# hsp-iit/roft

Measured on AMD Instinct MI355X. Metric: tracker frames/sec per object (640x480) + ADD-S vs CPU ref, higher is better.
Workload: dtype f64; 1 GPU; BASELINE config #4: 640x480, CV_32FC2 flow grid 1, 64 objects in total, 64 per GPU (sharded by object, no data-path collective; result rows all-gathered over RCCL at N > 1), masks+poses at 5 fps with 6-frame delay, flow-aided masks, re-sync and outlier rejection on, frames submitted in batches of at most 8; objects_per_gpu=64, objects_total=64, width=640, height=480, batch_frames=8, ranks=1, backend=nccl

## Files before the change

### include/roft_engine.h

```cpp
#ifndef ROFT_ENGINE_H
#define ROFT_ENGINE_H

#include <stddef.h>
#include <stdint.h>

#ifdef __cplusplus
extern "C" {
#endif

#define ROFT_ABI_VERSION 2

#define ROFT_OK 0
#define ROFT_ERR_INVALID (-1)
#define ROFT_ERR_DEVICE (-2)
#define ROFT_ERR_CAPACITY (-3)
#define ROFT_ERR_STATE (-4)

#define ROFT_FLOW_S16C2 11
#define ROFT_FLOW_F32C2 13

#define ROFT_MEAS_NONE 0
#define ROFT_MEAS_VELOCITY 1
#define ROFT_MEAS_POSE 2
#define ROFT_MEAS_POSE_VELOCITY 3
// ... 360 lines not shown

#define ROFT_SCENE_MAX_INSTANCES 256

typedef struct {
    int n_frames;
    int n_instances;
    const int* mesh_index;
    const double* poses;
    const uint8_t* valid;
    const uint8_t* background;
    int background_frames;
    int gray_background;
    const roft_scene_style* styles;
    int window_pixels;
} roft_scene_desc;

typedef struct roft_scene_renderer roft_scene_renderer;
int roft_scene_renderer_create(const roft_camera* cam, const roft_mesh* meshes, int n_meshes, int max_frames_per_call, int device,
                               roft_scene_renderer** out);
int roft_scene_renderer_destroy(roft_scene_renderer* r);
int roft_scene_render(roft_scene_renderer* r, const roft_scene_desc* desc, uint8_t* rgb_out, float* depth_out, int32_t* instance_out,
                      int32_t* triangle_out);
int roft_render_scene(const roft_camera* cam, const roft_mesh* meshes, int n_meshes, const roft_scene_desc* desc, uint8_t* rgb_out,
                      float* depth_out, int32_t* instance_out, int32_t* triangle_out);

int roft_debug_plan(const roft_config* cfg, const int* pose_valid, int n_frames, int* n_steps, int* n_corrections,
                    int* outlier, int* slots);
int roft_debug_restart_check(const roft_config* cfg, int n_objects, const int* has_mesh, const int* enrolled, int enrol_all,
                             const int* obj_ids, const roft_object_desc* descs, int n, int flags);
int roft_debug_probe_streams(roft_engine* e, double out[25]);
int roft_debug_sector_rate(int device, double* sectors_per_second);
int roft_debug_get_residency(roft_engine* e, unsigned long long out[32]);
int roft_debug_outlier_split(int mode);
int roft_debug_pose_errors_kernel_ms(double* ms_out);
int roft_debug_scene_kernel_ms(roft_scene_renderer* r, double ms_out[2]);
int roft_debug_depth_kernel_ms(roft_engine* e, double* ms_out);
int roft_debug_quality_kernel_ms(roft_engine* e, double* ms_out);
int roft_debug_pose_mask_kernel_ms(roft_engine* e, double* ms_out);
int roft_debug_get_dbg(roft_engine* e, int obj_id, long long out[32]);

#ifdef __cplusplus
}
#endif
#endif
```

### roft_amd/_lib.py

```python
import collections
import ctypes as C
import os
import subprocess

_HERE = os.path.dirname(os.path.abspath(__file__))
CSRC = os.path.join(_HERE, "csrc")
SO = os.environ.get("ROFT_LIB_SO") or os.path.join(CSRC, "libroft_hip.so")

OK = 0
ERR_INVALID, ERR_DEVICE, ERR_CAPACITY, ERR_STATE = -1, -2, -3, -4
FLOW_S16C2 = 11
FLOW_F32C2 = 13
MEAS_NONE, MEAS_VELOCITY, MEAS_POSE, MEAS_POSE_VELOCITY = 0, 1, 2, 3
MEM_HOST, MEM_DEVICE = 0, 1
RETAIN_FRAMES = 16
MAX_BATCH_FRAMES = 8
MAX_FLOW_CHASE = 30
RENDER_CONTRACT, RENDER_GL = 0, 1
ABI_VERSION = 2
POSE_ERROR_ADD, POSE_ERROR_ADDS = 0, 1
RESTART_KEEP_MESH = 1
LABEL_U8, LABEL_U16 = 1, 2
IMAGE_GRAY8, IMAGE_BGR8, IMAGE_RGB8 = 1, 2, 3
DEPTH_Z16 = 1
# ... 229 lines not shown
    Fn("roft_default_of_consistency", _int, [_P(OFConsistency)], _OPTIONAL),
    Fn("roft_optical_flow_checked", _int, [_vp, _vp, _int, _int, _P(OFParams), _P(OFConsistency), _vp], _OPTIONAL),
    Fn("roft_flow_producer_set_consistency", _int, [_vp, _P(OFConsistency)], _OPTIONAL),
    Fn("roft_engine_enable_flow_consistency", _int, [_vp, _P(OFConsistency)], _OPTIONAL),
    Fn("roft_engine_enable_raw_depth", _int, [_vp, _P(DepthSource)], _OPTIONAL),
    Fn("roft_engine_get_depth", _int, [_vp, _int, _vp], _OPTIONAL),
    Fn("roft_engine_get_depth_stats", _int, [_vp, _P(EngineDepthStats)], _OPTIONAL),
    Fn("roft_depth_convert", _int, [_vp, _int, _int, C.c_float, _vp], _OPTIONAL),
    Fn("roft_depth_align", _int, [_vp, _P(DepthSource), _P(Camera), _vp], _OPTIONAL),
    Fn("roft_default_quality_params", _int, [_P(QualityParams)], _OPTIONAL),
    Fn("roft_engine_enable_quality", _int, [_vp, _P(QualityParams)], _OPTIONAL),
    Fn("roft_engine_get_quality", _int, [_vp, _int, _int, _vp], _OPTIONAL),
    Fn("roft_track_quality", _int, [_P(Camera), _int, _vp, _vp, _P(Mesh), _vp, _vp, C.c_float, C.c_double, _int, _P(QualityRecord)], _OPTIONAL),
    Fn("roft_engine_enable_pose_masks", _int, [_vp, _ip, _int], _OPTIONAL),
    Fn("roft_engine_get_pose_mask_stats", _int, [_vp, _P(EnginePoseMaskStats)], _OPTIONAL),
    Fn("roft_pose_silhouette", _int, [_P(Camera), _P(Mesh), _vp, _vp, _int, _int, _vp, _ip], _OPTIONAL),
    Fn("roft_engine_enable_pose_mask_occlusion", _int, [_vp, _ip, _ip, _int], _OPTIONAL),
    Fn("roft_engine_get_pose_mask_occlusion_stats", _int, [_vp, _P(EnginePoseMaskOcclusionStats)], _OPTIONAL),
    Fn("roft_pose_silhouettes_occluded", _int, [_P(Camera), _P(Mesh), _int, _vp, _vp, _int, _int, _vp, _ip], _OPTIONAL),
    Fn("roft_default_pose_mask_gate", _int, [_P(PoseMaskGate)], _OPTIONAL),
    Fn("roft_engine_enable_pose_mask_depth_gate", _int, [_vp, _P(PoseMaskGate)], _OPTIONAL),
    Fn("roft_engine_get_pose_mask_gate_stats", _int, [_vp, _P(EnginePoseMaskGateStats)], _OPTIONAL),
    Fn("roft_pose_silhouettes_gated", _int, [_P(Camera), _P(Mesh), _int, _vp, _vp, _vp, _P(PoseMaskGate), _int, _int, _vp, _ip, _ip], _OPTIONAL),
    Fn("roft_scene_renderer_create", _int, [_P(Camera), _P(Mesh), _int, _int, _int, _P(_vp)], _OPTIONAL),
    Fn("roft_scene_renderer_destroy", _int, [_vp], _OPTIONAL),
    Fn("roft_scene_render", _int, [_vp, _P(SceneDesc), _vp, _vp, _vp, _vp], _OPTIONAL),
    Fn("roft_render_scene", _int, [_P(Camera), _P(Mesh), _int, _P(SceneDesc), _vp, _vp, _vp, _vp], _OPTIONAL),
    Fn("roft_debug_plan", _int, [_P(Config), _vp, _int, _vp, _vp, _vp, _vp], _OPTIONAL),
    Fn("roft_debug_restart_check", _int, [_P(Config), _int, _ip, _ip, _int, _ip, _P(ObjectDesc), _int, _int], _OPTIONAL),
    Fn("roft_debug_probe_streams", _int, [_vp, _dp], _OPTIONAL),
    Fn("roft_debug_sector_rate", _int, [_int, _dp], _OPTIONAL),
    Fn("roft_debug_get_residency", _int, [_vp, _P(C.c_ulonglong)], _OPTIONAL),
    Fn("roft_debug_outlier_split", _int, [_int], _OPTIONAL),
    Fn("roft_debug_pose_errors_kernel_ms", _int, [_dp], _OPTIONAL),
    Fn("roft_debug_scene_kernel_ms", _int, [_vp, _dp], _OPTIONAL),
    Fn("roft_debug_depth_kernel_ms", _int, [_vp, _dp], _OPTIONAL),
    Fn("roft_debug_quality_kernel_ms", _int, [_vp, _dp], _OPTIONAL),
    Fn("roft_debug_pose_mask_kernel_ms", _int, [_vp, _dp], _OPTIONAL),
    Fn("roft_debug_get_dbg", _int, [_vp, _int, _P(C.c_longlong)], _OPTIONAL),
)
ABI_SYMBOLS = [f.name for f in ABI]
NEWER_SYMBOLS = tuple(f.name for f in ABI if f.optional and not f.name.startswith("roft_debug_"))


def build(force=False):
    srcs = [os.path.join(CSRC, f) for f in os.listdir(CSRC) if f.endswith((".hip", ".h"))]
    srcs.append(os.path.join(_HERE, "..", "include", "roft_engine.h"))
    stale = (not os.path.exists(SO)) or any(os.path.getmtime(s) > os.path.getmtime(SO) for s in srcs)
    if force or stale:
        jobs = str(min(8, os.cpu_count() or 1))
        r = subprocess.run(["make", "-C", CSRC, "-j", jobs, "libroft_hip.so"], capture_output=True, text=True)
        if r.returncode != 0:
            raise RoftError("building libroft_hip.so failed:\n" + r.stdout[-4000:] + r.stderr[-4000:])
    return SO


_lib = None


def lib():
    global _lib
    if _lib is not None:
        return _lib
    if not os.path.exists(SO):
        build()
    L = C.CDLL(SO)
# ... 21 lines not shown
```

### roft_amd/csrc/engine_ops.hip

```cpp
#include "engine_internal.h"

namespace {

struct OpCtx {
    std::mutex mu;
    hipStream_t stream = nullptr;
    Arrays arr;
    int W = 0, H = 0, ftype = 0, fgrid = 0, radius = 0;
    DevBuf<unsigned char> b0, b1, b2, b3, b4, b5;
    DeviceMesh mesh;
    bool ready = false;

    int prepare(const roft_camera& cam, int ftype_, int fgrid_, float fscale, int radius_)
    {
        if (roft_device_count() <= 0) return fail(ROFT_ERR_DEVICE, "no HIP device (libroft_hip has no CPU path)");
        if (int rc = check_geometry(cam.width, cam.height)) return rc;
        HIP_TRY(hipSetDevice(0));
        (void)hipGetLastError();
        if (!stream) HIP_TRY(hipStreamCreateWithFlags(&stream, hipStreamNonBlocking));
        DevFlowFmt ff;
        ff.type = ftype_;
        ff.grid = std::max(fgrid_, 1);
        ff.cols = cam.width / ff.grid;
        ff.rows = cam.height / ff.grid;
// ... 544 lines not shown
    if (err != hipSuccess) { delete st; HIP_TRY(err); }
    c.arr.a.n_obj = 1;
    if (int rc = upload_ctrl(c, fc)) { delete st; return rc; }
    launch_ukf_chain(c.arr.a, *ut, true, 0, c.stream);
    err = hipMemcpyAsync(st, c.arr.state.p, sizeof(ObjState), hipMemcpyDeviceToHost, c.stream);
    if (err == hipSuccess) err = hipStreamSynchronize(c.stream);
    if (err == hipSuccess) err = hipGetLastError();
    if (err == hipSuccess) {
        std::memcpy(mean_out, st->belief[B_SPARE].mean, sizeof(double) * 13);
        std::memcpy(P_out, st->belief[B_SPARE].cov, sizeof(double) * 144);
        if (status) *status = st->lane[0].ukf_status & 0xF;
    }
    delete st;
    HIP_TRY(err);
    return ROFT_OK;
}

int roft_ukf_predict(const double mean[13], const double P[144], const double Q[81], double T, const roft_ut_params* ut,
                     double mean_out[13], double P_out[144])
{
    if (!mean || !P || !Q || !ut || !mean_out || !P_out) return fail(ROFT_ERR_INVALID, "null argument");
    return op_ukf(mean, P, Q, T, 0, nullptr, nullptr, ut, mean_out, P_out, nullptr);
}

int roft_ukf_correct(const double mean[13], const double P[144], int type, const double* meas, const double* Rdiag,
                     const roft_ut_params* ut, double mean_out[13], double P_out[144], int* status_out)
{
    if (!mean || !P || !ut || !mean_out || !P_out) return fail(ROFT_ERR_INVALID, "null argument");
    if (type != ROFT_MEAS_NONE && (!meas || !Rdiag)) return fail(ROFT_ERR_INVALID, "null measurement");
    if (type < ROFT_MEAS_NONE || type > ROFT_MEAS_POSE_VELOCITY) return fail(ROFT_ERR_INVALID, "bad measurement type");
    return op_ukf(mean, P, nullptr, 0.0, type, meas, Rdiag, ut, mean_out, P_out, status_out);
}

static int op_outlier(const roft_camera* cam, int divider, const float* depth, const uint8_t* mask, const roft_mesh* mesh,
                      const double* x2 , const double* q2 , const OutlierLaunchOpts& o_in, double L_out[2],
                      long samples_out[2], int* selected_out, float* tiles_out)
{
    TRY(check_mesh(*mesh, "mesh", false));
    OpCtx& c = op();
    std::lock_guard<std::mutex> lk(c.mu);
    if (int rc = c.prepare(*cam, ROFT_FLOW_F32C2, 1, 1.0f, 35)) return rc;
    EngineArrays& a = c.arr.a;
    a.cam.divider = divider;
    a.tile_w = cam->width / divider;
    a.tile_h = cam->height / divider;
    const size_t npix = (size_t)cam->width * cam->height, tpix = (size_t)a.tile_w * a.tile_h;
    if (int rc = c.arr.ensure_zmerge(1, tpix)) return rc;
    auto restore = [&]() {
        a.cam = make_cam(*cam);
        a.tile_w = cam->width / a.cam.divider;
        a.tile_h = cam->height / a.cam.divider;
        a.max_verts = a.max_tris = 0;
        a.meshes_without_clusters = 0;
    };
    TRY(c.mesh.upload(*mesh, o_in.render_mode == ROFT_RENDER_CONTRACT ? MeshLayout::kWalkClusters : MeshLayout::kAsItIs, c.stream));
    ObjParams prm;
    std::memset(&prm, 0, sizeof(prm));
    c.mesh.describe(prm);
    a.max_verts = mesh->n_verts;
    a.max_tris = mesh->n_tris;
    a.meshes_without_clusters = (prm.n_tris > 0 && prm.n_clusters <= 0) ? 1 : 0;
    FrameCtrl fc;
    clear_ctrl(fc);
    fc.n_steps = 1;
    fc.outlier_step = 0;
    fc.cur_slot = B_LIN0;
// ... 18 lines not shown
        PoseBelief& b = st->belief[b_alt(0, k)];
        for (int i = 0; i < 3; ++i) b.mean[6 + i] = x2[3 * k + i];
        for (int i = 0; i < 4; ++i) b.mean[9 + i] = q2[4 * k + i];
    }
    hipError_t err = hipMemcpyAsync(c.arr.state.p, st, sizeof(ObjState), hipMemcpyHostToDevice, c.stream);
    if (err == hipSuccess) err = hipMemcpyAsync(c.arr.params.p, &prm, sizeof(prm), hipMemcpyHostToDevice, c.stream);
    if (err == hipSuccess) err = hipStreamSynchronize(c.stream);
    if (err != hipSuccess) { delete st; restore(); HIP_TRY(err); }
    if (int rc = upload_ctrl(c, fc)) { delete st; restore(); return rc; }
    OutlierLaunchOpts o = o_in;
    if (tiles_out) {
        err = c.b4.ensure(sizeof(float) * 2 * tpix);
        if (err == hipSuccess) err = hipMemsetAsync(c.b4.p, 0, sizeof(float) * 2 * tpix, c.stream);
        if (err != hipSuccess) { delete st; restore(); HIP_TRY(err); }
        o.tile_dump = reinterpret_cast<float*>(c.b4.p);
    }
    if (depth && mask) {
        launch_mask_ingest(a, 0, c.stream);
        launch_features(a, c.stream);
    }
    TRY(launch_outlier(a, 0, c.stream, nullptr, &o));
    roft_ut_params ut{1.0, 2.0, 0.0};
    launch_ukf_chain(a, ut, false, 0, c.stream);
    err = hipMemcpyAsync(st, c.arr.state.p, sizeof(ObjState), hipMemcpyDeviceToHost, c.stream);
    if (err == hipSuccess && tiles_out) err = hipMemcpyAsync(tiles_out, c.b4.p, sizeof(float) * 2 * tpix, hipMemcpyDeviceToHost, c.stream);
    if (err == hipSuccess) err = hipStreamSynchronize(c.stream);
    if (err == hipSuccess) err = hipGetLastError();
    if (err == hipSuccess) {
        for (int k = 0; k < 2; ++k) {
            if (L_out) L_out[k] = st->lane[0].outlier_L[k];
            if (samples_out) samples_out[k] = (long)st->lane[0].outlier_cnt[k];
        }
        if (selected_out) *selected_out = st->lane[0].outlier_selected;
    }
    delete st;
    restore();
    HIP_TRY(err);
    return ROFT_OK;
}

int roft_mesh_classify(const roft_mesh* mesh, uint8_t* flip_out, int* closed_out)
{
    if (!mesh || !mesh->verts || !mesh->tris || !has_mesh(*mesh) || !closed_out) return fail(ROFT_ERR_INVALID, "bad argument");
    std::vector<uint8_t> flip;
    *closed_out = classify_mesh(mesh->verts, mesh->n_verts, mesh->tris, mesh->n_tris, flip) ? 1 : 0;
    if (flip_out) std::memcpy(flip_out, flip.data(), (size_t)mesh->n_tris);
    return ROFT_OK;
}

int roft_render_depth(const roft_mesh* mesh, const double x[3], const double q[4], const roft_camera* cam, int divider,
                      float* tile)
{
    return roft_render_depth_mode(mesh, x, q, cam, divider, ROFT_RENDER_CONTRACT, tile);
}

int roft_render_depth_mode(const roft_mesh* mesh, const double x[3], const double q[4], const roft_camera* cam, int divider, int mode,
                           float* tile)
{
    if (!mesh || !x || !q || !cam || !tile || divider <= 0) return fail(ROFT_ERR_INVALID, "bad argument");
    if (mode != ROFT_RENDER_CONTRACT && mode != ROFT_RENDER_GL) return fail(ROFT_ERR_INVALID, "bad render mode");
    const size_t tpix = (size_t)(cam->width / divider) * (cam->height / divider);
    std::vector<float> tiles(2 * tpix);
    const double x2[6] = {x[0], x[1], x[2], x[0], x[1], x[2]};
    const double q2[8] = {q[0], q[1], q[2], q[3], q[0], q[1], q[2], q[3]};
    OutlierLaunchOpts o;
    o.render_mode = mode;
    if (int rc = op_outlier(cam, divider, nullptr, nullptr, mesh, x2, q2, o, nullptr, nullptr, nullptr, tiles.data())) return rc;
    std::memcpy(tile, tiles.data(), sizeof(float) * tpix);
    return ROFT_OK;
}
// ... 124 lines not shown
```

### roft_amd/csrc/k_render.hip

```cpp
#include <algorithm>
#include <atomic>
#include <string>

#include "mesh_clusters.h"
#include "plane_rank.h"
#include "raster.h"

namespace roft {

namespace host { int fail(int code, const std::string& msg); }

constexpr int kFeatThreads = 1024;

#ifdef ROFT_FEAT_PROFILE
#define FTICK(i) do { __syncthreads(); if (threadIdx.x == 0) { long long _t = wall_clock64(); a.state[obj].dbg[i] = _t - f_t0; f_t0 = _t; } } while (0)
#else
#define FTICK(i) do {} while (0)
#endif

template <bool LDS>
__global__ __launch_bounds__(kFeatThreads) void features_kernel(EngineArrays a, unsigned frames_packed)
{
    ROFT_RESIDENT(a, RK_FEATURES);
    extern __shared__ __attribute__((aligned(16))) unsigned char smem[];
// ... 238 lines not shown
        pl.outlier_L[0] = L[0];
        pl.outlier_L[1] = L[1];
        for (int k = 0; k < 2; ++k) {
            double n2 = 0.0;
            for (int w = 0; w < kOutlierThreads / 64; ++w) n2 += s_cnt[k][w];
            pl.outlier_cnt[k] = n2;
        }
        s_sel = sel;
    }
    __syncthreads();
    const PoseBelief& src = st.belief[b_alt(lin, s_sel ? 1 : 0)];
    PoseBelief& dst = st.belief[c.cur_slot];
    for (int i = threadIdx.x; i < 144; i += blockDim.x) dst.cov[i] = src.cov[i];
    if (threadIdx.x < 13) dst.mean[threadIdx.x] = src.mean[threadIdx.x];
    if (roft_object_output* row = log_row(a, c, obj)) {
        if (threadIdx.x < 13) row->pose[threadIdx.x] = src.mean[threadIdx.x];
        if (threadIdx.x == 0) {
            row->outlier_selected = s_sel;
            row->outlier_L[0] = pl.outlier_L[0];
            row->outlier_L[1] = pl.outlier_L[1];
        }
    }
}

constexpr int kFusedThreads = 1024;
#ifdef ROFT_FUSED_PROFILE
#define UTICK(i) do { __syncthreads(); if (threadIdx.x == 0 && bx < 4) { long long _t = wall_clock64(); st.dbg[bx * 8 + (i)] += _t - u_t0; u_t0 = _t; } } while (0)
#else
#define UTICK(i) do {} while (0)
#endif

template <bool GL>
__global__ __launch_bounds__(kFusedThreads) void outlier_fused_kernel(EngineArrays a, int lin, int vcache_cap, int win_cap, int parts,
                                                                     int split_tris, float* tile_dump)
{
    ROFT_RESIDENT(a, RK_OUTLIER);
    extern __shared__ __attribute__((aligned(16))) unsigned char smem[];
    __shared__ long long s_hi[kFusedThreads / 64], s_lo[kFusedThreads / 64];
    __shared__ int s_cnt[kFusedThreads / 64];
    __shared__ int s_box[4];
    __shared__ int s_behind;
    __shared__ int s_last;
    __shared__ int s_settled;
    const int per = 2 * parts, lin_id = (int)blockIdx.x;
    const int obj = (lin_id / (8 * per)) * 8 + (lin_id & 7), bx = (lin_id >> 3) % per;
    if (obj >= a.n_obj) return;
    const int alt = bx / parts, part = bx % parts, tid = threadIdx.x;
    ObjState& st = a.state[obj];
    PoseLane& pl = st.lane[lin];
    if (pl.pending_frame < 0) return;
    const FrameCtrl& c = frame_ctrl(a, pl.pending_frame, obj);
    const ObjParams& prm = a.params[obj];
    const PoseBelief& bl = st.belief[b_alt(lin, alt)];
    const RenderPose P = make_pose(bl.mean + 6, bl.mean + 9);
    const int d = a.cam.divider, tw = a.tile_w, th = a.tile_h;
    const float fx = (float)(a.cam.fx / d), fy = (float)(a.cam.fy / d), cx = (float)(a.cam.cx / d), cy = (float)(a.cam.cy / d);
    const int nv = prm.n_verts, nt = prm.n_tris;
    const bool cached = GL && nv <= vcache_cap;
    float* s_v = reinterpret_cast<float*>(smem);
    uint32_t* s_z = reinterpret_cast<uint32_t*>(smem + (GL ? vertex_cache_bytes(vcache_cap) : 0));
    uint64_t* s_k = reinterpret_cast<uint64_t*>(s_z);
    if (tid < 4) s_box[tid] = (tid < 2) ? INT32_MAX : -1;
    if (tid == 0) s_behind = 0;
#ifdef ROFT_FUSED_PROFILE
    long long u_t0 = wall_clock64();
    if (tid < 8 && bx < 4) st.dbg[bx * 8 + tid] = 0;
#endif
    __syncthreads();
    auto project = [&](const float* v, float& sx, float& sy, float& z) {
        if constexpr (GL) project_vertex_gl(v, P, fx, fy, cx, cy, sx, sy, z);
        else project_vertex(v, P, fx, fy, cx, cy, sx, sy, z);
    };
    if constexpr (GL) {
        project_mesh<kFusedThreads, 4>(prm.verts, nv, cached, s_v, tw, th, s_box, &s_behind, project);
        __syncthreads();
    } else {
        if (tid < 64 && prm.n_clusters > 0) {
            const int k = tid & 7;
            const float vc[3] = {prm.box_corners[3 * k], prm.box_corners[3 * k + 1], prm.box_corners[3 * k + 2]};
            int box[4];
            const bool settled = corner_box_settles(vc, P, fx, fy, cx, cy, tw, th, box);
            if (tid == 0) {
                s_settled = settled ? 1 : 0;
                if (settled) { s_box[0] = box[0]; s_box[1] = box[1]; s_box[2] = box[2]; s_box[3] = box[3]; }
            }
        } else if (tid == 0) {
            s_settled = 1;
        }
        __syncthreads();
        if (!s_settled) {
            project_mesh<kFusedThreads, 4>(prm.verts, nv, false, s_v, tw, th, s_box, &s_behind, project);
            __syncthreads();
        }
    }
    UTICK(0);
    const int i0 = min(s_box[0], tw - 1), i1 = s_box[2];
    int j0 = min(s_box[1], th - 1), j1 = s_box[3];
    int R = parts;
    if (!GL && split_tris && parts > 1 && i1 >= i0 && j1 >= j0 && i0 >= 0 && j0 >= 0) {
        const long long w_all = i1 - i0 + 1, rows_all = j1 - j0 + 1;
        for (R = 1; R < parts; ++R)
            if (parts % R == 0 && ((rows_all + R - 1) / R) * w_all <= (long long)win_cap) break;
    }
    const int G = parts / R, band = part / G, grp = part % G;
    const bool split = G > 1;
    if (j1 >= j0 && R > 1) {
        const int rows_all = j1 - j0 + 1, b0 = j0 + (int)((long long)rows_all * band / R), b1 = j0 + (int)((long long)rows_all * (band + 1) / R) - 1;
        j0 = b0;
        j1 = b1;
    }
    const int win_w = i1 - i0 + 1;
    const int fslot = (c.feat_read >= 0) ? c.feat_read : 0;
    const uint32_t* fpix = a.feat_pix + ((size_t)obj * kFeatRing + fslot) * a.feat_cap;
    const float* fdep = a.feat_depth + ((size_t)obj * kFeatRing + fslot) * a.feat_cap;
    const int n = st.n_feat[fslot];
    LikelihoodSum err;
    int cnt = 0;
    auto gl_resolve = [&](uint64_t key, int i, int j) -> float {
        const int32_t* tri = prm.tris + (size_t)3 * (uint32_t)key;
        const int v0 = tri[0], v1 = tri[1], v2 = tri[2];
        float x0, y0, z0, x1, y1, z1, x2, y2, z2;
        fetch_triangle(s_v, cached, prm.verts, v0, v1, v2, project, x0, y0, z0, x1, y1, z1, x2, y2, z2);
        return gl_linear_depth(gl_pixel_window_z(x0, y0, x1, y1, x2, y2, gl_vertex_window_z(z0), gl_vertex_window_z(z1),
                                                 gl_vertex_window_z(z2), (float)i + 0.5f, (float)j + 0.5f));
    };
    if (win_w > 0 && j1 >= j0 && i0 >= 0 && j0 >= 0) {
        const int rows = max(1, win_cap / win_w);
        for (int js = j0; js <= j1; js += rows) {
            const int je = min(j1, js + rows - 1), npx = win_w * (je - js + 1);
            if constexpr (GL) {
                for (int i = tid; i < npx; i += kFusedThreads) s_k[i] = kGlKeyClear;
            } else {
                for (int i = tid; i < npx; i += kFusedThreads) s_z[i] = kDepthEmpty;
            }
            __syncthreads();
            UTICK(1);
            ROFT_LDS uint32_t* const zw = pin_lds(s_z);
            auto store = [zw, i0, js, win_w](int i, int j, float z) {
                (void)__hip_atomic_fetch_min(zw + ((j - js) * win_w + (i - i0)), __float_as_uint(z), __ATOMIC_RELAXED, __HIP_MEMORY_SCOPE_WORKGROUP);
            };
            ROFT_LDS uint64_t* const zk = (ROFT_LDS uint64_t*)zw;
            auto store_key = [zk, i0, js, win_w](int i, int j, uint64_t key) {
                (void)__hip_atomic_fetch_min(zk + ((j - js) * win_w + (i - i0)), key, __ATOMIC_RELAXED, __HIP_MEMORY_SCOPE_WORKGROUP);
            };
            if constexpr (GL) {
                constexpr int kTB = 8;
                for (int tb = tid; tb < nt; tb += kTB * kFusedThreads) {
                    int idx[kTB][3];
#pragma unroll
                    for (int k = 0; k < kTB; ++k) {
                        const int32_t* tri = prm.tris + (size_t)3 * min(tb + k * kFusedThreads, nt - 1);
                        idx[k][0] = tri[0]; idx[k][1] = tri[1]; idx[k][2] = tri[2];
                    }
#pragma unroll
                    for (int k = 0; k < kTB; ++k) {
                        if (tb + k * kFusedThreads >= nt) break;
                        float x0, y0, z0, x1, y1, z1, x2, y2, z2;
                        fetch_triangle(s_v, cached, prm.verts, idx[k][0], idx[k][1], idx[k][2], project, x0, y0, z0, x1, y1, z1, x2, y2, z2);
                        const uint64_t t = (uint32_t)(tb + k * kFusedThreads);
                        raster_projected_gl(x0, y0, z0, x1, y1, z1, x2, y2, z2, tw, th, js, je,
                                            [&](int i, int j, uint32_t qz) { store_key(i, j, ((uint64_t)qz << 32) | t); });
                    }
                }
            } else {
                const bool rule_on = cull_table(prm.tri_flip, s_behind) != nullptr;
                const bool cones = rule_on && fx > 0.0f && fy > 0.0f && pose_is_rotation(P.R);
                const float f_lo = fminf(fx, fy), f_hi = fmaxf(fx, fy), c_abs = fabsf(cx) + fabsf(cy);
                const int lane = tid & 63, wave = __builtin_amdgcn_readfirstlane(tid >> 6);
                const int nc = prm.n_clusters, n_waves = kFusedThreads / 64;
                auto cluster_of = [=](int i) { return (i * n_waves + wave) * G + grp; };
                auto fetch = [&](int c, float (&v)[3], uint32_t& w) {
                    const float* sl = prm.cl_slots + (size_t)c * 3 * kClusterSize + lane;
                    v[0] = sl[0]; v[1] = sl[kClusterSize]; v[2] = sl[2 * kClusterSize];
                    w = prm.cl_words[(size_t)c * kClusterSize + lane];
                };
                for (int base = 0; cluster_of(base) < nc; base += 64) {
                    const int mine = cluster_of(base + lane);
                    bool live = mine < nc;
                    if (live && cones) {
                        const uint4* hp = reinterpret_cast<const uint4*>(prm.cl_headers + (size_t)mine * kClusterWords);
                        const uint4 h0 = hp[0], h1 = hp[1], h2 = hp[2], h3 = hp[3];
                        static_assert(kCwCone == 2 && kCwAxis == 4 && kCwCos == 7 && kCwSin == 8 && kCwCenter == 9 && kCwRadius == 12 &&
                                      kCwAreaMin == 13 && kCwEdgeMax == 14, "the header words as they are unpacked here");
                        if (h0.z && cluster_faces_away(__uint_as_float(h1.x), __uint_as_float(h1.y), __uint_as_float(h1.z), __uint_as_float(h1.w),
                                                       __uint_as_float(h2.x), __uint_as_float(h2.y), __uint_as_float(h2.z), __uint_as_float(h2.w),
                                                       __uint_as_float(h3.x), __uint_as_float(h3.y), __uint_as_float(h3.z), P.R, P.t, f_lo, f_hi, c_abs))
                            live = false;
                    }
                    unsigned long long todo = __ballot(live);
                    if (!todo) continue;
                    float v[3];
                    uint32_t w;
                    fetch(cluster_of(base + (int)__builtin_ctzll(todo)), v, w);
                    while (todo) {
                        todo &= todo - 1;
                        float v_n[3] = {v[0], v[1], v[2]};
                        uint32_t w_n = w;
                        if (todo) fetch(cluster_of(base + (int)__builtin_ctzll(todo)), v_n, w_n);
                        float sx, sy, z;
                        project_vertex(v, P, fx, fy, cx, cy, sx, sy, z);
                        const int a0 = (int)(w & 63u), a1 = (int)((w >> 6) & 63u), a2 = (int)((w >> 12) & 63u);
                        const float x0 = __shfl(sx, a0, 64), y0 = __shfl(sy, a0, 64), z0 = __shfl(z, a0, 64);
                        const float x1 = __shfl(sx, a1, 64), y1 = __shfl(sy, a1, 64), z1 = __shfl(z, a1, 64);
                        const float x2 = __shfl(sx, a2, 64), y2 = __shfl(sy, a2, 64), z2 = __shfl(z, a2, 64);
                        raster_projected(x0, y0, z0, x1, y1, z1, x2, y2, z2, tw, th, js, je, rule_on ? 1 + (int)((w >> 18) & 1u) : 0, store);
                        v[0] = v_n[0]; v[1] = v_n[1]; v[2] = v_n[2];
                        w = w_n;
                    }
                }
            }
            __syncthreads();
            UTICK(2);
            if constexpr (!GL) if (split) {
                const size_t slab0 = (((size_t)lin * a.zmerge_slabs + (size_t)obj * parts + (size_t)band * G) * 2 + alt) * a.zmerge_stride;
                uint32_t* mine = a.zmerge + slab0 + (size_t)grp * 2 * a.zmerge_stride;
                int* arrivals = a.zcount + (((size_t)lin * a.n_obj + obj) * 2 + alt) * kMaxOutlierParts + band;
                for (int i = tid; i < npx; i += kFusedThreads)
                    __hip_atomic_store(&mine[i], s_z[i], __ATOMIC_RELAXED, __HIP_MEMORY_SCOPE_AGENT);
                __atomic_signal_fence(__ATOMIC_SEQ_CST);
                __builtin_amdgcn_s_waitcnt(0);
                __atomic_signal_fence(__ATOMIC_SEQ_CST);
                __syncthreads();
                if (tid == 0) {
                    const int before = __hip_atomic_fetch_add(arrivals, 1, __ATOMIC_RELAXED, __HIP_MEMORY_SCOPE_AGENT);
                    s_last = (before == G - 1) ? 1 : 0;
                    if (before == G - 1) __hip_atomic_store(arrivals, 0, __ATOMIC_RELAXED, __HIP_MEMORY_SCOPE_AGENT);
                }
                __syncthreads();
                if (!s_last) return;
                static_assert(kMaxOutlierParts <= 8, "eight slabs per pixel");
                const uint32_t* others = a.zmerge + slab0;
                const size_t slab_step = 2 * a.zmerge_stride;
                const uint32_t* op[7];
                {
                    int k = 0;
#pragma unroll
                    for (int p = 0; p < 8; ++p)
                        if (p < G && p != grp && k < 7) op[k++] = others + (size_t)p * slab_step;
                    for (; k < 7; ++k) op[k] = others;
                }
                for (int i = tid; i < npx; i += kFusedThreads) {
                    uint32_t m = s_z[i];
                    uint32_t v0, v1, v2, v3, v4, v5, v6;
                    switch (G - 1) {
                    case 1:
                        asm volatile("global_load_dword %0, %1, off sc1\n\ts_waitcnt vmcnt(0)" : "=&v"(v0) : "v"(op[0] + i) : "memory");
                        m = min(m, v0);
                        break;
                    case 2:
                        asm volatile("global_load_dword %0, %2, off sc1\n\tglobal_load_dword %1, %3, off sc1\n\ts_waitcnt vmcnt(0)"
                                     : "=&v"(v0), "=&v"(v1) : "v"(op[0] + i), "v"(op[1] + i) : "memory");
                        m = min(m, min(v0, v1));
                        break;
                    case 3:
                        asm volatile("global_load_dword %0, %3, off sc1\n\tglobal_load_dword %1, %4, off sc1\n\tglobal_load_dword %2, %5, off sc1\n\t"
                                     "s_waitcnt vmcnt(0)"
                                     : "=&v"(v0), "=&v"(v1), "=&v"(v2) : "v"(op[0] + i), "v"(op[1] + i), "v"(op[2] + i) : "memory");
                        m = min(min(m, v0), min(v1, v2));
                        break;
                    case 4:
                        asm volatile("global_load_dword %0, %4, off sc1\n\tglobal_load_dword %1, %5, off sc1\n\tglobal_load_dword %2, %6, off sc1\n\t"
                                     "global_load_dword %3, %7, off sc1\n\ts_waitcnt vmcnt(0)"
                                     : "=&v"(v0), "=&v"(v1), "=&v"(v2), "=&v"(v3) : "v"(op[0] + i), "v"(op[1] + i), "v"(op[2] + i), "v"(op[3] + i) : "memory");
                        m = min(m, min(min(v0, v1), min(v2, v3)));
                        break;
                    default:
                        asm volatile("global_load_dword %0, %7, off sc1\n\tglobal_load_dword %1, %8, off sc1\n\tglobal_load_dword %2, %9, off sc1\n\t"
                                     "global_load_dword %3, %10, off sc1\n\tglobal_load_dword %4, %11, off sc1\n\tglobal_load_dword %5, %12, off sc1\n\t"
                                     "global_load_dword %6, %13, off sc1\n\ts_waitcnt vmcnt(0)"
                                     : "=&v"(v0), "=&v"(v1), "=&v"(v2), "=&v"(v3), "=&v"(v4), "=&v"(v5), "=&v"(v6)
                                     : "v"(op[0] + i), "v"(op[1] + i), "v"(op[2] + i), "v"(op[3] + i), "v"(op[4] + i), "v"(op[5] + i), "v"(op[6] + i) : "memory");
                        m = min(min(m, v0), min(min(v1, v2), min(min(v3, v4), min(v5, v6))));
                        break;
                    case 0: break;
                    }
                    s_z[i] = m;
                }
                __syncthreads();
            }
            if (tile_dump) {
                float* tile = tile_dump + (size_t)alt * tw * th;
                if constexpr (GL) {
                    for (int i = tid; i < npx; i += kFusedThreads) {
                        const uint64_t key = s_k[i];
                        const int pi = i0 + i % win_w, pj = js + i / win_w;
                        tile[(size_t)pj * tw + pi] = ((uint32_t)(key >> 32) == kGlDepthClear) ? 0.0f : gl_resolve(key, pi, pj);
                    }
                } else {
                    for (int i = tid; i < npx; i += kFusedThreads) {
                        const uint32_t b = s_z[i];
                        tile[(size_t)(js + i / win_w) * tw + (i0 + i % win_w)] = (b == kDepthEmpty) ? 0.0f : __uint_as_float(b);
                    }
                }
            }
            constexpr int kBatch = 16;
            for (int f0 = tid; f0 < n; f0 += kBatch * kFusedThreads) {
                float dep[kBatch];
                uint32_t pix[kBatch];
#pragma unroll
                for (int k = 0; k < kBatch; ++k) {
                    const int i = f0 + k * kFusedThreads;
                    dep[k] = (i < n) ? fdep[i] : 0.0f;
                    pix[k] = (i < n) ? fpix[i] : 0u;
                }
#pragma unroll
                for (int k = 0; k < kBatch; ++k) {
                    if (!((dep[k] > 0) && ((double)dep[k] < 2.0))) continue;
                    const int v = (int)(pix[k] >> 16), u = (int)(pix[k] & 0xFFFFu);
                    const int tj = v / d, ti = u / d;
                    if (tj < js || tj > je || ti < i0 || ti > i1) continue;
                    if constexpr (GL) {
// ... 25 lines not shown
        long long hi = 0, lo = 0;
        int n2 = 0;
        for (int w = 0; w < kFusedThreads / 64; ++w) { hi += s_hi[w]; lo += s_lo[w]; n2 += s_cnt[w]; }
        pl.part_hi[alt][band] = hi;
        pl.part_lo[alt][band] = lo;
        pl.part_cnt[alt][band] = (double)n2;
        if (band == 0) pl.n_parts[alt] = R;
    }
}

static std::atomic<int> g_outlier_split{-1};
void set_outlier_split(int mode) { g_outlier_split.store(mode < 0 ? -1 : (mode ? 1 : 0), std::memory_order_relaxed); }

int launch_outlier(const EngineArrays& a, int lin, hipStream_t s, hipEvent_t stop, const OutlierLaunchOpts* opts)
{
    if (!(opts && opts->render_mode == ROFT_RENDER_GL) && a.meshes_without_clusters > 0)
        return host::fail(ROFT_ERR_STATE, "outlier test: a mesh went up without clusters (MeshLayout::kWalkClusters)");
    const size_t lds_total = kRasterLdsBudget;
    const size_t vbytes = vertex_cache_bytes(a.max_verts);
    const bool gl = opts && opts->render_mode == ROFT_RENDER_GL;
    const size_t zb = gl ? 8 : 4;
    const size_t min_win = zb * std::max(8192, a.tile_w);
    const bool cache = gl && vbytes + min_win <= lds_total && !(opts && opts->no_vertex_cache);
    const int vcache_cap = cache ? a.max_verts : 0;
    int win_cap = (int)((lds_total - (cache ? vbytes : 0)) / zb);
    (void)set_max_dynamic_lds(gl ? reinterpret_cast<const void*>(outlier_fused_kernel<true>) : reinterpret_cast<const void*>(outlier_fused_kernel<false>),
                              (int)lds_total);
    int parts = std::max(1, std::min(kMaxOutlierParts, device_cu_count() / (2 * std::max(a.n_obj, 1))));
    if (a.outlier_parts > 0) parts = std::min(a.outlier_parts, kMaxOutlierParts);
    if (opts && opts->parts > 0) parts = std::min(opts->parts, kMaxOutlierParts);
    if (opts && opts->parts < 0) parts = std::max(1, parts / -opts->parts);
    static const int split_env = getenv("ROFT_OUTLIER_SPLIT") ? atoi(getenv("ROFT_OUTLIER_SPLIT")) : -1;
    const int forced = g_outlier_split.load(std::memory_order_relaxed) >= 0 ? g_outlier_split.load(std::memory_order_relaxed) : split_env;
    int split = (opts && opts->split >= 0) ? opts->split : (forced >= 0 ? forced : 1);
    if (parts <= 1 || !a.zmerge || (size_t)a.n_obj * parts > a.zmerge_slabs) split = 0;
    if (gl) split = 0;
    const int lds_parts = split ? 1 : parts;
    const size_t win_need = zb * std::max((size_t)a.tile_w, ((size_t)a.tile_w * a.tile_h + lds_parts - 1) / lds_parts + (size_t)a.tile_w);
    const size_t lds = std::min(lds_total, (((cache ? vbytes : 0) + win_need + 15) & ~(size_t)15));
    win_cap = std::min(win_cap, (int)((lds - (cache ? vbytes : 0)) / zb));
    if (opts && opts->window_pixels > 0) win_cap = std::max(a.tile_w, std::min(win_cap, opts->window_pixels));
    if (gl)
        hipExtLaunchKernelGGL(outlier_fused_kernel<true>, dim3(2 * parts * ((a.n_obj + 7) / 8) * 8), dim3(kFusedThreads), (uint32_t)lds, s, nullptr, stop, 0, a,
                              lin, vcache_cap, win_cap, parts, split, opts ? opts->tile_dump : nullptr);
    else
        hipExtLaunchKernelGGL(outlier_fused_kernel<false>, dim3(2 * parts * ((a.n_obj + 7) / 8) * 8), dim3(kFusedThreads), (uint32_t)lds, s, nullptr, stop, 0, a,
                              lin, vcache_cap, win_cap, parts, split, opts ? opts->tile_dump : nullptr);
    return ROFT_OK;
}

void launch_outlier_only(const EngineArrays& a, hipStream_t s)
{
    hipLaunchKernelGGL(outlier_kernel, dim3(a.n_obj), dim3(kOutlierThreads), 0, s, a, 0);
}

}
```

### roft_amd/csrc/mesh_clusters.h

```cpp
#pragma once

#include <algorithm>
#include <cmath>
#include <cstdint>
#include <cstring>
#include <limits>
#include <vector>

#if defined(__HIPCC__)
#define ROFT_CLUSTER_HD __host__ __device__
#else
#define ROFT_CLUSTER_HD
#endif

namespace roft {

constexpr int kClusterSize = 64;
constexpr int kClusterWords = 16;
enum ClusterWord {
    kCwVerts = 0, kCwTris = 1, kCwCone = 2 , kCwBucket = 3,
    kCwAxis = 4 , kCwCos = 7, kCwSin = 8, kCwCenter = 9 , kCwRadius = 12, kCwAreaMin = 13, kCwEdgeMax = 14,
};

ROFT_CLUSTER_HD inline uint32_t pack_cluster_triangle(int s0, int s1, int s2, int flip)
{
    return (uint32_t)s0 | ((uint32_t)s1 << 6) | ((uint32_t)s2 << 12) | ((uint32_t)(flip ? 1 : 0) << 18);
}

ROFT_CLUSTER_HD inline bool cluster_faces_away(float ax0, float ax1, float ax2, float cos_t, float sin_t, float c0, float c1, float c2,
                                               float radius, float a_min, float e_max, const float* R, const float* t, float f_lo,
                                               float f_hi, float c_abs)
{
    const float vx = ((R[0] * c0 + R[1] * c1) + R[2] * c2) + t[0];
    const float vy = ((R[3] * c0 + R[4] * c1) + R[5] * c2) + t[1];
    const float vz = ((R[6] * c0 + R[7] * c1) + R[8] * c2) + t[2];
    const float ex = (R[0] * ax0 + R[1] * ax1) + R[2] * ax2;
    const float ey = (R[3] * ax0 + R[4] * ax1) + R[5] * ax2;
    const float ez = (R[6] * ax0 + R[7] * ax1) + R[8] * ax2;
    const float L = sqrtf((vx * vx + vy * vy) + vz * vz);
    const float D = L + radius, Z = vz - radius;
    const float Dm = fmaxf(D, (fabsf(c0) + fabsf(c1) + fabsf(c2)) + 1.75f * radius + fmaxf(fabsf(t[0]), fmaxf(fabsf(t[1]), fabsf(t[2]))));
    if (!(Z > 0.0f) || !(L > 0.0f)) return false;
    float cphi = ((vx * ex + vy * ey) + vz * ez) / L;
    cphi = fminf(fmaxf(cphi, -1.0f), 1.0f);
    const float sphi = sqrtf(fmaxf(0.0f, 1.0f - cphi * cphi));
    const float m = L * (cphi * cos_t - sphi * sin_t) - radius - 2.4e-5f * Dm;
    if (!(m > 0.0f)) return false;
    const float q = D / Z;
    const float d = 1e-6f * (f_hi * (Dm / Z) * (1.0f + q)) + 2e-7f * c_abs;
    const float edge = f_hi * e_max * 1.4143f * q / Z;
    const float lhs = f_lo * f_lo * a_min * m / (D * D * D);
    const float rhs = 2.0f * (8.0f * d * edge + 8.0f * d * d + 8.0f * 6e-8f * edge * edge);
    return lhs >= rhs;
}

ROFT_CLUSTER_HD inline bool pose_is_rotation(const float* R)
{
    bool ok = true;
    for (int i = 0; i < 3; ++i)
        for (int j = i; j < 3; ++j) {
            const float g = (R[3 * i] * R[3 * j] + R[3 * i + 1] * R[3 * j + 1]) + R[3 * i + 2] * R[3 * j + 2];
            ok = ok && fabsf(g - (i == j ? 1.0f : 0.0f)) <= 2e-6f;
        }
    const float det = (R[0] * (R[4] * R[8] - R[5] * R[7]) - R[1] * (R[3] * R[8] - R[5] * R[6])) + R[2] * (R[3] * R[7] - R[4] * R[6]);
    return ok && det > 0.0f;
}

struct MeshClusters {
    int n_clusters = 0;
    std::vector<uint32_t> headers;
    std::vector<float> slots;
    std::vector<uint32_t> words;
    float box[8][3];
    std::vector<int32_t> tri_index;
    std::vector<int32_t> slot_vertex;
};

inline uint32_t cluster_float_bits(float f)
{
    uint32_t u;
    std::memcpy(&u, &f, 4);
    return u;
}

inline void build_clusters(const float* verts, int n_verts, const int32_t* tris, int n_tris, const uint8_t* flip, const uint8_t* bucket,
                           MeshClusters& out)
// ... 82 lines not shown
        take(seed);
        while (nt < kClusterSize) {
            int best = -1, best_fresh = 4;
            double best_d2 = 0.0;
            size_t keep = 0;
            for (size_t i = 0; i < frontier.size(); ++i) {
                const int u = frontier[i];
                if (done[u]) continue;
                frontier[keep++] = u;
                const int fresh = fresh_corners(u);
                if (nv + fresh > kClusterSize) continue;
                double d2 = 0.0;
                for (int q = 0; q < 3; ++q) {
                    const double dq = centroid[(size_t)3 * u + q] - centroid[(size_t)3 * seed + q];
                    d2 += dq * dq;
                }
                if (fresh < best_fresh || (fresh == best_fresh && (d2 < best_d2 || (d2 == best_d2 && u < best)))) { best = u; best_fresh = fresh; best_d2 = d2; }
            }
            frontier.resize(keep);
            if (best < 0 && frontier.empty()) {
                int u = cursor;
                while (u < b1 && done[u]) ++u;
                if (u < b1 && nv + fresh_corners(u) <= kClusterSize) best = u;
            }
            if (best < 0) break;
            take(best);
        }
        for (int sl = nv; sl < kClusterSize; ++sl)
            for (int q = 0; q < 3; ++q) out.slots[((size_t)c * 3 + q) * kClusterSize + sl] = out.slots[((size_t)c * 3 + q) * kClusterSize];
        uint32_t* h = out.headers.data() + (size_t)c * kClusterWords;
        h[kCwVerts] = (uint32_t)nv;
        h[kCwTris] = (uint32_t)nt;
        h[kCwBucket] = bucket ? bucket[seed] : 0u;
        if (!flip) continue;
        double sum[3] = {0, 0, 0}, a_min = std::numeric_limits<double>::infinity(), e_max = 0.0;
        std::vector<double> normals((size_t)3 * nt);
        bool ok = true;
        for (int k = 0; k < nt && ok; ++k) {
            const int32_t* tri = tris + (size_t)3 * members[k];
            const float *a = verts + (size_t)3 * tri[0], *b = verts + (size_t)3 * tri[1], *cc = verts + (size_t)3 * tri[2];
            const double e1[3] = {(double)b[0] - a[0], (double)b[1] - a[1], (double)b[2] - a[2]};
            const double e2[3] = {(double)cc[0] - a[0], (double)cc[1] - a[1], (double)cc[2] - a[2]};
            const double e3[3] = {(double)cc[0] - b[0], (double)cc[1] - b[1], (double)cc[2] - b[2]};
            double n[3] = {e1[1] * e2[2] - e1[2] * e2[1], e1[2] * e2[0] - e1[0] * e2[2], e1[0] * e2[1] - e1[1] * e2[0]};
            const double len = std::sqrt(n[0] * n[0] + n[1] * n[1] + n[2] * n[2]);
            if (!(len > 0.0) || !std::isfinite(len)) { ok = false; break; }
            const double sgn = flip[members[k]] ? -1.0 : 1.0;
            for (int q = 0; q < 3; ++q) { normals[(size_t)3 * k + q] = sgn * n[q] / len; sum[q] += sgn * n[q] / len; }
            a_min = std::min(a_min, len);
            for (const double* e : {e1, e2, e3}) e_max = std::max(e_max, std::sqrt(e[0] * e[0] + e[1] * e[1] + e[2] * e[2]));
        }
        const double sl = std::sqrt(sum[0] * sum[0] + sum[1] * sum[1] + sum[2] * sum[2]);
        if (!ok || !(sl > 1e-6 * nt)) continue;
        const float axis[3] = {(float)(sum[0] / sl), (float)(sum[1] / sl), (float)(sum[2] / sl)};
        double cos_t = 1.0;
        for (int k = 0; k < nt; ++k)
            cos_t = std::min(cos_t, normals[(size_t)3 * k] * axis[0] + normals[(size_t)3 * k + 1] * axis[1] + normals[(size_t)3 * k + 2] * axis[2]);
        cos_t -= 1e-6;
        if (!(cos_t > 1e-3)) continue;
        const double sin_t = std::sqrt(std::max(0.0, 1.0 - cos_t * cos_t)) * (1.0 + 1e-6) + 1e-7;
        float clo[3], chi[3], center[3];
        for (int q = 0; q < 3; ++q) {
            clo[q] = chi[q] = out.slots[((size_t)c * 3 + q) * kClusterSize];
            for (int s2 = 1; s2 < nv; ++s2) {
                clo[q] = std::min(clo[q], out.slots[((size_t)c * 3 + q) * kClusterSize + s2]);
                chi[q] = std::max(chi[q], out.slots[((size_t)c * 3 + q) * kClusterSize + s2]);
            }
            center[q] = 0.5f * clo[q] + 0.5f * chi[q];
        }
        double r2 = 0.0;
        for (int s2 = 0; s2 < nv; ++s2) {
            double d2 = 0.0;
            for (int q = 0; q < 3; ++q) {
                const double dq = (double)out.slots[((size_t)c * 3 + q) * kClusterSize + s2] - center[q];
                d2 += dq * dq;
            }
            r2 = std::max(r2, d2);
        }
        const float radius = (float)(std::sqrt(r2) * (1.0 + 1e-6)), f_amin = (float)(a_min * (1.0 - 1e-6)), f_emax = (float)(e_max * (1.0 + 1e-6));
        if (!std::isfinite(radius) || !(f_amin > 0.0f) || !std::isfinite(f_emax) || !std::isfinite(center[0] + center[1] + center[2])) continue;
        h[kCwCone] = 1u;
        for (int q = 0; q < 3; ++q) { h[kCwAxis + q] = cluster_float_bits(axis[q]); h[kCwCenter + q] = cluster_float_bits(center[q]); }
        h[kCwCos] = cluster_float_bits((float)cos_t);
        h[kCwSin] = cluster_float_bits((float)sin_t);
        h[kCwRadius] = cluster_float_bits(radius);
        h[kCwAreaMin] = cluster_float_bits(f_amin);
        h[kCwEdgeMax] = cluster_float_bits(f_emax);
      }
      b0 = b1;
    }
}

}
```

Before: 1.791 million object-frames/s.

## Cull mesh clusters by bounding sphere against row bands in outlier render

Stores a bounding sphere for every mesh cluster, not only for cone-eligible clusters, and adds a conservative test that drops clusters whose projected sphere misses the current row band of the split outlier render. It also forces a minimum number of row bands when parts is at most 2, so that per-band culling can take effect. The aim is to rasterise fewer triangles per band. The cost is an extra header load and sphere projection per cluster, and possibly more bands and more merge work. A debug entry point for the band counts and timing ticks is added too.

```diff
diff --git a/include/roft_engine.h b/include/roft_engine.h
--- a/include/roft_engine.h
+++ b/include/roft_engine.h
@@ -416,6 +416,7 @@
 int roft_debug_sector_rate(int device, double* sectors_per_second);
 int roft_debug_get_residency(roft_engine* e, unsigned long long out[32]);
 int roft_debug_outlier_split(int mode);
+int roft_debug_outlier_last_bands(int bands_out[2], int* arrivals_out);
 int roft_debug_pose_errors_kernel_ms(double* ms_out);
 int roft_debug_scene_kernel_ms(roft_scene_renderer* r, double ms_out[2]);
 int roft_debug_depth_kernel_ms(roft_engine* e, double* ms_out);
diff --git a/roft_amd/_lib.py b/roft_amd/_lib.py
--- a/roft_amd/_lib.py
+++ b/roft_amd/_lib.py
@@ -285,6 +285,7 @@
     Fn("roft_debug_sector_rate", _int, [_int, _dp], _OPTIONAL),
     Fn("roft_debug_get_residency", _int, [_vp, _P(C.c_ulonglong)], _OPTIONAL),
     Fn("roft_debug_outlier_split", _int, [_int], _OPTIONAL),
+    Fn("roft_debug_outlier_last_bands", _int, [_ip, _ip], _OPTIONAL),
     Fn("roft_debug_pose_errors_kernel_ms", _int, [_dp], _OPTIONAL),
     Fn("roft_debug_scene_kernel_ms", _int, [_vp, _dp], _OPTIONAL),
     Fn("roft_debug_depth_kernel_ms", _int, [_vp, _dp], _OPTIONAL),
diff --git a/roft_amd/csrc/engine_ops.hip b/roft_amd/csrc/engine_ops.hip
--- a/roft_amd/csrc/engine_ops.hip
+++ b/roft_amd/csrc/engine_ops.hip
@@ -600,6 +600,8 @@
     return op_ukf(mean, P, nullptr, 0.0, type, meas, Rdiag, ut, mean_out, P_out, status_out);
 }
 
+static int g_last_bands[2] = {0, 0};
+
 static int op_outlier(const roft_camera* cam, int divider, const float* depth, const uint8_t* mask, const roft_mesh* mesh,
                       const double* x2 , const double* q2 , const OutlierLaunchOpts& o_in, double L_out[2],
                       long samples_out[2], int* selected_out, float* tiles_out)
@@ -684,10 +686,27 @@
             if (samples_out) samples_out[k] = (long)st->lane[0].outlier_cnt[k];
         }
         if (selected_out) *selected_out = st->lane[0].outlier_selected;
+        for (int k = 0; k < 2; ++k) g_last_bands[k] = st->lane[0].n_parts[k];
     }
     delete st;
     restore();
     HIP_TRY(err);
+    return ROFT_OK;
+}
+
+int roft_debug_outlier_last_bands(int bands_out[2], int* arrivals_out)
+{
+    if (!bands_out || !arrivals_out) return fail(ROFT_ERR_INVALID, "null argument");
+    OpCtx& c = op();
+    std::lock_guard<std::mutex> lk(c.mu);
+    bands_out[0] = g_last_bands[0];
+    bands_out[1] = g_last_bands[1];
+    *arrivals_out = 0;
+    if (c.arr.zcount.p && c.arr.zcount.n > 0) {
+        std::vector<int> counts(c.arr.zcount.n);
+        HIP_TRY(hipMemcpy(counts.data(), c.arr.zcount.p, sizeof(int) * counts.size(), hipMemcpyDeviceToHost));
+        for (int v : counts) *arrivals_out += v != 0 ? 1 : 0;
+    }
     return ROFT_OK;
 }
 
diff --git a/roft_amd/csrc/k_render.hip b/roft_amd/csrc/k_render.hip
--- a/roft_amd/csrc/k_render.hip
+++ b/roft_amd/csrc/k_render.hip
@@ -294,7 +294,7 @@
 
 template <bool GL>
 __global__ __launch_bounds__(kFusedThreads) void outlier_fused_kernel(EngineArrays a, int lin, int vcache_cap, int win_cap, int parts,
-                                                                     int split_tris, float* tile_dump)
+                                                                     int split_tris, int min_bands, float* tile_dump)
 {
     ROFT_RESIDENT(a, RK_OUTLIER);
     extern __shared__ __attribute__((aligned(16))) unsigned char smem[];
@@ -358,10 +358,11 @@
     UTICK(0);
     const int i0 = min(s_box[0], tw - 1), i1 = s_box[2];
     int j0 = min(s_box[1], th - 1), j1 = s_box[3];
+    const int j0_all = j0, j1_all = j1;
     int R = parts;
     if (!GL && split_tris && parts > 1 && i1 >= i0 && j1 >= j0 && i0 >= 0 && j0 >= 0) {
         const long long w_all = i1 - i0 + 1, rows_all = j1 - j0 + 1;
-        for (R = 1; R < parts; ++R)
+        for (R = max(1, min(min_bands, parts)); R < parts; ++R)
             if (parts % R == 0 && ((rows_all + R - 1) / R) * w_all <= (long long)win_cap) break;
     }
     const int G = parts / R, band = part / G, grp = part % G;
@@ -426,7 +427,9 @@
                 }
             } else {
                 const bool rule_on = cull_table(prm.tri_flip, s_behind) != nullptr;
-                const bool cones = rule_on && fx > 0.0f && fy > 0.0f && pose_is_rotation(P.R);
+                const bool rigid = fy > 0.0f && pose_is_rotation(P.R);
+                const bool cones = rule_on && fx > 0.0f && rigid;
+                const bool row_cull = rigid && (js > j0_all || je < j1_all);
                 const float f_lo = fminf(fx, fy), f_hi = fmaxf(fx, fy), c_abs = fabsf(cx) + fabsf(cy);
                 const int lane = tid & 63, wave = __builtin_amdgcn_readfirstlane(tid >> 6);
                 const int nc = prm.n_clusters, n_waves = kFusedThreads / 64;
@@ -439,14 +442,17 @@
                 for (int base = 0; cluster_of(base) < nc; base += 64) {
                     const int mine = cluster_of(base + lane);
                     bool live = mine < nc;
-                    if (live && cones) {
+                    if (live && (cones || row_cull)) {
                         const uint4* hp = reinterpret_cast<const uint4*>(prm.cl_headers + (size_t)mine * kClusterWords);
                         const uint4 h0 = hp[0], h1 = hp[1], h2 = hp[2], h3 = hp[3];
                         static_assert(kCwCone == 2 && kCwAxis == 4 && kCwCos == 7 && kCwSin == 8 && kCwCenter == 9 && kCwRadius == 12 &&
-                                      kCwAreaMin == 13 && kCwEdgeMax == 14, "the header words as they are unpacked here");
-                        if (h0.z && cluster_faces_away(__uint_as_float(h1.x), __uint_as_float(h1.y), __uint_as_float(h1.z), __uint_as_float(h1.w),
-                                                       __uint_as_float(h2.x), __uint_as_float(h2.y), __uint_as_float(h2.z), __uint_as_float(h2.w),
-                                                       __uint_as_float(h3.x), __uint_as_float(h3.y), __uint_as_float(h3.z), P.R, P.t, f_lo, f_hi, c_abs))
+                                      kCwAreaMin == 13 && kCwEdgeMax == 14 && kCwSphere == 15, "the header words as they are unpacked here");
+                        if (row_cull && h3.w && cluster_misses_rows(__uint_as_float(h2.y), __uint_as_float(h2.z), __uint_as_float(h2.w), __uint_as_float(h3.x),
+                                                                    P.R, P.t, fy, cy, js, je))
+                            live = false;
+                        else if (cones && h0.z && cluster_faces_away(__uint_as_float(h1.x), __uint_as_float(h1.y), __uint_as_float(h1.z), __uint_as_float(h1.w),
+                                                                     __uint_as_float(h2.x), __uint_as_float(h2.y), __uint_as_float(h2.z), __uint_as_float(h2.w),
+                                                                     __uint_as_float(h3.x), __uint_as_float(h3.y), __uint_as_float(h3.z), P.R, P.t, f_lo, f_hi, c_abs))
                             live = false;
                     }
                     unsigned long long todo = __ballot(live);
@@ -489,6 +495,7 @@
                     if (before == G - 1) __hip_atomic_store(arrivals, 0, __ATOMIC_RELAXED, __HIP_MEMORY_SCOPE_AGENT);
                 }
                 __syncthreads();
+                UTICK(7);
                 if (!s_last) return;
                 static_assert(kMaxOutlierParts <= 8, "eight slabs per pixel");
                 const uint32_t* others = a.zmerge + slab0;
@@ -539,6 +546,7 @@
                     s_z[i] = m;
                 }
                 __syncthreads();
+                UTICK(7);
             }
             if (tile_dump) {
                 float* tile = tile_dump + (size_t)alt * tw * th;
@@ -630,9 +638,13 @@
     if (opts && opts->parts < 0) parts = std::max(1, parts / -opts->parts);
     static const int split_env = getenv("ROFT_OUTLIER_SPLIT") ? atoi(getenv("ROFT_OUTLIER_SPLIT")) : -1;
     const int forced = g_outlier_split.load(std::memory_order_relaxed) >= 0 ? g_outlier_split.load(std::memory_order_relaxed) : split_env;
-    int split = (opts && opts->split >= 0) ? opts->split : (forced >= 0 ? forced : 1);
+    const int asked = (opts && opts->split >= 0) ? opts->split : forced;
+    int split = asked >= 0 ? asked : 1;
     if (parts <= 1 || !a.zmerge || (size_t)a.n_obj * parts > a.zmerge_slabs) split = 0;
     if (gl) split = 0;
+    static const int min_bands_env = getenv("ROFT_OUTLIER_MIN_BANDS") ? atoi(getenv("ROFT_OUTLIER_MIN_BANDS")) : 0;
+    int min_bands = 1;
+    if (asked < 0) min_bands = min_bands_env > 0 ? min_bands_env : (parts <= 2 ? parts : 1);
     const int lds_parts = split ? 1 : parts;
     const size_t win_need = zb * std::max((size_t)a.tile_w, ((size_t)a.tile_w * a.tile_h + lds_parts - 1) / lds_parts + (size_t)a.tile_w);
     const size_t lds = std::min(lds_total, (((cache ? vbytes : 0) + win_need + 15) & ~(size_t)15));
@@ -640,10 +652,10 @@
     if (opts && opts->window_pixels > 0) win_cap = std::max(a.tile_w, std::min(win_cap, opts->window_pixels));
     if (gl)
         hipExtLaunchKernelGGL(outlier_fused_kernel<true>, dim3(2 * parts * ((a.n_obj + 7) / 8) * 8), dim3(kFusedThreads), (uint32_t)lds, s, nullptr, stop, 0, a,
-                              lin, vcache_cap, win_cap, parts, split, opts ? opts->tile_dump : nullptr);
+                              lin, vcache_cap, win_cap, parts, split, min_bands, opts ? opts->tile_dump : nullptr);
     else
         hipExtLaunchKernelGGL(outlier_fused_kernel<false>, dim3(2 * parts * ((a.n_obj + 7) / 8) * 8), dim3(kFusedThreads), (uint32_t)lds, s, nullptr, stop, 0, a,
-                              lin, vcache_cap, win_cap, parts, split, opts ? opts->tile_dump : nullptr);
+                              lin, vcache_cap, win_cap, parts, split, min_bands, opts ? opts->tile_dump : nullptr);
     return ROFT_OK;
 }
 
diff --git a/roft_amd/csrc/mesh_clusters.h b/roft_amd/csrc/mesh_clusters.h
--- a/roft_amd/csrc/mesh_clusters.h
+++ b/roft_amd/csrc/mesh_clusters.h
@@ -20,6 +20,7 @@
 enum ClusterWord {
     kCwVerts = 0, kCwTris = 1, kCwCone = 2 , kCwBucket = 3,
     kCwAxis = 4 , kCwCos = 7, kCwSin = 8, kCwCenter = 9 , kCwRadius = 12, kCwAreaMin = 13, kCwEdgeMax = 14,
+    kCwSphere = 15 ,
 };
 
 ROFT_CLUSTER_HD inline uint32_t pack_cluster_triangle(int s0, int s1, int s2, int flip)
@@ -52,6 +53,26 @@
     const float lhs = f_lo * f_lo * a_min * m / (D * D * D);
     const float rhs = 2.0f * (8.0f * d * edge + 8.0f * d * d + 8.0f * 6e-8f * edge * edge);
     return lhs >= rhs;
+}
+
+ROFT_CLUSTER_HD inline bool cluster_misses_rows(float c0, float c1, float c2, float radius, const float* R, const float* t, float fy, float cy,
+                                                int js, int je)
+{
+    const float vx = ((R[0] * c0 + R[1] * c1) + R[2] * c2) + t[0];
+    const float vy = ((R[3] * c0 + R[4] * c1) + R[5] * c2) + t[1];
+    const float vz = ((R[6] * c0 + R[7] * c1) + R[8] * c2) + t[2];
+    const float D = sqrtf((vx * vx + vy * vy) + vz * vz) + radius;
+    const float Dm = fmaxf(D, (fabsf(c0) + fabsf(c1) + fabsf(c2)) + 1.75f * radius + fmaxf(fabsf(t[0]), fmaxf(fabsf(t[1]), fabsf(t[2]))));
+    const float r = radius + 1e-5f * Dm;
+    const float Z = vz - r, far = vz + r;
+    if (!(radius >= 0.0f) || !(Z > 0.01f * far)) return false;
+    const float den = Z * far;
+    const float rs = r * sqrtf(vy * vy + den), yz = vy * vz;
+    const float kmag = (fabsf(yz) + rs) / den;
+    const float k_hi = (yz + rs) / den + 2e-5f * kmag, k_lo = (yz - rs) / den - 2e-5f * kmag;
+    const float d = 2e-6f * ((fy * kmag + fabsf(cy)) + 1.0f);
+    const float hi = (fy * k_hi + cy) + d, lo = (fy * k_lo + cy) - d;
+    return hi < (float)js + 0.5f || lo > (float)je + 0.5f;
 }
 
 ROFT_CLUSTER_HD inline bool pose_is_rotation(const float* R)
@@ -200,6 +221,31 @@
         h[kCwVerts] = (uint32_t)nv;
         h[kCwTris] = (uint32_t)nt;
         h[kCwBucket] = bucket ? bucket[seed] : 0u;
+        float clo[3], chi[3], center[3];
+        for (int q = 0; q < 3; ++q) {
+            clo[q] = chi[q] = out.slots[((size_t)c * 3 + q) * kClusterSize];
+            for (int s2 = 1; s2 < nv; ++s2) {
+                clo[q] = std::min(clo[q], out.slots[((size_t)c * 3 + q) * kClusterSize + s2]);
+                chi[q] = std::max(chi[q], out.slots[((size_t)c * 3 + q) * kClusterSize + s2]);
+            }
+            center[q] = 0.5f * clo[q] + 0.5f * chi[q];
+        }
+        double r2 = 0.0;
+        bool all_finite = true;
+        for (int s2 = 0; s2 < nv; ++s2) {
+            double d2 = 0.0;
+            for (int q = 0; q < 3; ++q) {
+                const double dq = (double)out.slots[((size_t)c * 3 + q) * kClusterSize + s2] - center[q];
+                all_finite = all_finite && std::isfinite(dq);
+                d2 += dq * dq;
+            }
+            r2 = std::max(r2, d2);
+        }
+        const float radius = (float)(std::sqrt(r2) * (1.0 + 1e-6));
+        if (!all_finite || !std::isfinite(radius) || !std::isfinite(center[0]) || !std::isfinite(center[1]) || !std::isfinite(center[2])) continue;
+        h[kCwSphere] = 1u;
+        for (int q = 0; q < 3; ++q) h[kCwCenter + q] = cluster_float_bits(center[q]);
+        h[kCwRadius] = cluster_float_bits(radius);
         if (!flip) continue;
         double sum[3] = {0, 0, 0}, a_min = std::numeric_limits<double>::infinity(), e_max = 0.0;
         std::vector<double> normals((size_t)3 * nt);
@@ -227,31 +273,12 @@
         cos_t -= 1e-6;
         if (!(cos_t > 1e-3)) continue;
         const double sin_t = std::sqrt(std::max(0.0, 1.0 - cos_t * cos_t)) * (1.0 + 1e-6) + 1e-7;
-        float clo[3], chi[3], center[3];
-        for (int q = 0; q < 3; ++q) {
-            clo[q] = chi[q] = out.slots[((size_t)c * 3 + q) * kClusterSize];
-            for (int s2 = 1; s2 < nv; ++s2) {
-                clo[q] = std::min(clo[q], out.slots[((size_t)c * 3 + q) * kClusterSize + s2]);
-                chi[q] = std::max(chi[q], out.slots[((size_t)c * 3 + q) * kClusterSize + s2]);
-            }
-            center[q] = 0.5f * clo[q] + 0.5f * chi[q];
-        }
-        double r2 = 0.0;
-        for (int s2 = 0; s2 < nv; ++s2) {
-            double d2 = 0.0;
-            for (int q = 0; q < 3; ++q) {
-                const double dq = (double)out.slots[((size_t)c * 3 + q) * kClusterSize + s2] - center[q];
-                d2 += dq * dq;
-            }
-            r2 = std::max(r2, d2);
-        }
-        const float radius = (float)(std::sqrt(r2) * (1.0 + 1e-6)), f_amin = (float)(a_min * (1.0 - 1e-6)), f_emax = (float)(e_max * (1.0 + 1e-6));
-        if (!std::isfinite(radius) || !(f_amin > 0.0f) || !std::isfinite(f_emax) || !std::isfinite(center[0] + center[1] + center[2])) continue;
+        const float f_amin = (float)(a_min * (1.0 - 1e-6)), f_emax = (float)(e_max * (1.0 + 1e-6));
+        if (!(f_amin > 0.0f) || !std::isfinite(f_emax)) continue;
         h[kCwCone] = 1u;
-        for (int q = 0; q < 3; ++q) { h[kCwAxis + q] = cluster_float_bits(axis[q]); h[kCwCenter + q] = cluster_float_bits(center[q]); }
+        for (int q = 0; q < 3; ++q) h[kCwAxis + q] = cluster_float_bits(axis[q]);
         h[kCwCos] = cluster_float_bits((float)cos_t);
         h[kCwSin] = cluster_float_bits((float)sin_t);
-        h[kCwRadius] = cluster_float_bits(radius);
         h[kCwAreaMin] = cluster_float_bits(f_amin);
         h[kCwEdgeMax] = cluster_float_bits(f_emax);
       }
```

Measured after the change: 1.791 million object-frames/s (median of 2 runs). No clear change (+0.0%).
